# maxvonbuelow/harry

Measured on AMD Instinct MI355X. Metric: Mtriangles/s encode+decode, higher is better.
Workload: dtype u8/u16 residual bytes, u32 range-coder registers (compat profile: u64)

## Files before the change

### harry_amd/csrc/device/chunked.cpp

```cpp
#include <chrono>
#include <condition_variable>
#include <cstdio>
#include <cstdlib>
#include <cstring>
#include <deque>
#include <memory>
#include <mutex>
#include <thread>

#include "codec_math.hpp"
#include "context.hpp"
#include "kernels.hpp"

namespace hry {

using namespace dev;
static const char kMarkPrefix[] = "[hry enc]";

static constexpr int kDefaultChunk = 8192;
static constexpr uint32_t kMaxChunk = 1u << 20;


static uint32_t stream_words(uint32_t n, uint32_t t0)
{
// ... 596 lines not shown
	build_init_tables(m, kind_tabs);
	const uint32_t CHC = std::min(CH, std::max(CH / 8, 512u));
	dir.CH = CH; dir.CHC = CHC;
	const uint32_t npl = (uint32_t)planes.size();
	std::vector<HistSlice> slices;
	for (uint32_t pi = 0; pi < npl; ++pi)
		for (uint32_t f = 0; f < planes[pi].n; f += 16384) slices.push_back(HistSlice{ planes[pi].dptr + f, std::min(16384u, planes[pi].n - f), pi });
	cx.d_small.ensure(std::max<size_t>(slices.size() * sizeof(HistSlice) + (size_t)npl * 1024 + 64, 64));
	uint32_t *d_hist = cx.d_small.as<uint32_t>();
	HistSlice *d_slices = (HistSlice*)(cx.d_small.as<uint8_t>() + (size_t)npl * 1024);
	if (!slices.empty()) HIP_OK(hipMemcpyAsync(d_slices, slices.data(), slices.size() * sizeof(HistSlice), hipMemcpyHostToDevice, cx.stream));
	HIP_OK(hipMemsetAsync(d_hist, 0, (size_t)npl * 1024, cx.stream));
	HIP_OK(hipStreamSynchronize(cx.stream));
	cx.timing.h2d_ms = ms_since(t_h2d);
	HRY_MARK(t_all, "walk's outputs on the device");

	ConnView cv = cx.conn_view();
	HIP_OK(hipEventRecord(cx.ev[1], cx.stream));
	if (!m.general && !piped) {
		HIP_OK(hipMemsetAsync(cx.d_rank.p, 0xff, (size_t)dev_nv * 4, cx.stream));
		launch_rank(cx.stream, cx.d_order_v.as<uint32_t>(), vc, cv.org, cx.d_rank.as<uint32_t>());
		launch_predict_vtx(cx.stream, cv, cx.d_order_v.as<uint32_t>(), vc, cx.d_rank.as<uint32_t>(), cx.d_rec[1].as<uint8_t>(), ldv, cx.d_vplanes.as<uint8_t>());
		launch_face_planes(cx.stream, cv, cx.d_order_f.as<uint32_t>(), fc, cx.d_rec[0].as<uint8_t>(), ldf, cx.d_fplanes.as<uint8_t>());
	}
	split_conn_groups(cx, w, !nt_piped);
	{
		uint32_t base[8], o = 0;
		for (int k = 0; k < 8; ++k) { base[k] = o; o += (uint32_t)op_plane_n[k]; }
		cx.d_op.ensure(((nopb + kSplitUnit - 1) / kSplitUnit + 1) * 8 * 4 + 64);
		launch_split_classes(cx.stream, d_opraw, (uint32_t)nopb, base, cx.d_op.as<uint32_t>(), d_opplanes);
	}
	launch_plane_hist(cx.stream, d_slices, (uint32_t)slices.size(), d_hist);
	HIP_OK(hipEventRecord(cx.ev[2], cx.stream));
	std::vector<uint32_t> hist((size_t)npl * 256);
	if (npl) HIP_OK(hipMemcpyAsync(hist.data(), d_hist, hist.size() * 4, hipMemcpyDeviceToHost, cx.stream));
	HIP_OK(hipStreamSynchronize(cx.stream));
	HRY_MARK(t_all, "planes and their histograms");

	dir.tables.assign((size_t)npl * 256, 0);
	dir.has_prior.assign(npl, 0);
	dir.nsym.resize(npl);
	std::vector<uint32_t> totals(npl, 0);
	for (uint32_t pi = 0; pi < npl; ++pi) {
		uint32_t *tab = dir.tables.data() + (size_t)pi * 256;
		const bool use = plane_prior_from_hist(hist.data() + (size_t)pi * 256, planes[pi].n, tab);
		if (!use) memcpy(tab, kind_tabs.data() + (size_t)planes[pi].init * 256, 1024);
		for (int i = 0; i < 256; ++i) totals[pi] += tab[i];
		dir.has_prior[pi] = use ? 1 : 0;
		dir.nsym[pi] = planes[pi].n;
	}
	std::vector<StreamJob> jobs;
	uint64_t words = 0;
	uint64_t nsym_total = 0;
	uint32_t max_t0 = 256;
	for (uint32_t pi = 0; pi < npl; ++pi) {
		const PlaneRef &pl = planes[pi];
		nsym_total += pl.n;
		max_t0 = std::max(max_t0, totals[pi]);
		for_plane_streams(pi, pl.n, CH, CHC, [&](uint64_t f, uint32_t n) {
			if (words >= (1ull << 32) - (1u << 24)) throw Error(HRY_E_UNSUPPORTED, "chunked stream accumulator exceeds 2^32 words");
			jobs.push_back(StreamJob{ pl.dptr + f, n, pi, totals[pi], (uint32_t)words });
			words += stream_words(n, totals[pi]);
		});
	}
	const uint32_t ns = (uint32_t)jobs.size();
	const uint32_t nw = (uint32_t)words + 2;
	HRY_MARK(t_all, "  priors and stream jobs (host)");
	cx.d_init.ensure(std::max<size_t>(dir.tables.size() * 4, 16));
	if (!dir.tables.empty()) HIP_OK(hipMemcpyAsync(cx.d_init.p, dir.tables.data(), dir.tables.size() * 4, hipMemcpyHostToDevice, cx.stream));
	cx.d_cjobs.ensure(std::max<size_t>((size_t)ns * sizeof(StreamJob), 16));
	if (ns) HIP_OK(hipMemcpyAsync(cx.d_cjobs.p, jobs.data(), (size_t)ns * sizeof(StreamJob), hipMemcpyHostToDevice, cx.stream));
	cx.ensure_magic(max_t0 + CH + 16);
	cx.d_acc.ensure((size_t)nw * 8);
	cx.d_summary.ensure(((size_t)nw / 1024 + 8) * 4);
	cx.d_bytes.ensure((size_t)nw * 4);
	cx.d_csizes.ensure(std::max<size_t>((size_t)ns * 8, 16));
	cx.d_coffs.ensure(((size_t)ns + 1) * 8);
	HIP_OK(hipMemsetAsync(cx.d_acc.p, 0, (size_t)nw * 8, cx.stream));
	uint32_t *d_bits = cx.d_csizes.as<uint32_t>(), *d_nbytes = d_bits + ns;
	bool split_kernels;
	{
		uint32_t longest = 0;
		for (uint32_t i = 0; i < ns; ++i) longest = std::max(longest, jobs[i].n);
		const double one = std::max(longest * 0.09e-3, (double)nsym_total * 0.04e-6), two = longest * 0.207e-3 + (double)nsym_total * 0.0057e-6;
		const uint64_t min_streams = env_uint("HRY_ENCODE_SPLIT_MIN_STREAMS", ~0ull);
		split_kernels = min_streams != ~0ull ? min_streams != 0 && ns >= min_streams : ns >= 64 && two < 0.9 * one;
	}
	for (uint32_t i = 0; i < ns && split_kernels; ++i) split_kernels = (uint64_t)jobs[i].t0 + jobs[i].n <= 65535u;
	std::vector<uint64_t> tab;
	if (split_kernels) {
		tab.resize((size_t)ns + ((size_t)ns + 1) / 2);
		uint32_t *order = (uint32_t*)(tab.data() + ns);
		uint64_t off = 0;
		for (uint32_t i = 0; i < ns; ++i) { tab[i] = off; off += jobs[i].n; order[i] = i; }
		std::stable_sort(order, order + ns, [&](uint32_t a, uint32_t b) { return jobs[a].n > jobs[b].n; });
		cx.d_rec_sym.ensure(std::max<size_t>((size_t)off * 8, 16));
		cx.d_split.ensure(tab.size() * 8);
		HIP_OK(hipMemcpyAsync(cx.d_split.p, tab.data(), tab.size() * 8, hipMemcpyHostToDevice, cx.stream));
		HIP_OK(hipEventRecord(cx.ev[3], cx.stream));
		launch_chunk_encode_split(cx.stream, cx.d_cjobs.as<StreamJob>(), ns, cx.d_init.as<uint32_t>(), cx.d_magic.as<MagicEnt>(), cx.d_acc.as<uint64_t>(), d_bits,
		                          cx.d_split.as<uint64_t>(), cx.d_rec_sym.p, (const uint32_t*)(cx.d_split.as<uint64_t>() + ns));
		HIP_OK(hipEventRecord(cx.ev[4], cx.stream));
	} else {
	HIP_OK(hipEventRecord(cx.ev[3], cx.stream));
	launch_chunk_encode(cx.stream, cx.d_cjobs.as<StreamJob>(), ns, cx.d_init.as<uint32_t>(), cx.d_magic.as<MagicEnt>(), cx.d_acc.as<uint64_t>(), d_bits);
	HIP_OK(hipEventRecord(cx.ev[4], cx.stream));
	}
	launch_carry(cx.stream, cx.d_acc.as<uint64_t>(), nw, cx.d_v.as<uint64_t>(), cx.d_summary.as<uint32_t>(), cx.d_bytes.as<uint8_t>(), cx.d_cjobs.as<StreamJob>(), d_bits, ns);
	launch_stream_pack(cx.stream, cx.d_cjobs.as<StreamJob>(), ns, d_bits, nullptr, d_nbytes, cx.d_coffs.as<uint64_t>(), nullptr, false);
	cx.h_small.ensure(64);
	volatile uint64_t *total_bytes_p = cx.h_small.as<uint64_t>();
	*total_bytes_p = 0;
	HIP_OK(hipMemcpyAsync((void*)total_bytes_p, cx.d_coffs.as<uint64_t>() + ns, 8, hipMemcpyDeviceToHost, cx.stream));
	HRY_MARK(t_all, "  stream kernels launched");
	if (dir_beside) dir_helper.rethrow(); else select_restarts();
	HRY_MARK(t_all, "  restart points selected");
	HIP_OK(hipStreamSynchronize(cx.stream));
	const uint64_t total_bytes = *total_bytes_p;
	HRY_MARK(t_all, "streams coded");
	cx.d_cout.ensure(std::max<size_t>(total_bytes, 16));
	launch_stream_pack(cx.stream, cx.d_cjobs.as<StreamJob>(), ns, d_bits, cx.d_bytes.as<uint8_t>(), d_nbytes, cx.d_coffs.as<uint64_t>(), cx.d_cout.as<uint8_t>(), true);
	HIP_OK(hipEventRecord(cx.ev[5], cx.stream));

	write_container(cx, dir, restart_sec, ns, d_nbytes, total_bytes, out);
	HRY_MARK(t_all, "container on the host");
	if (sharded) { const uint64_t seg_len = out.size() - seg_begin; memcpy(out.data() + seg_len_at, &seg_len, 8); }
	if (cx.want_order) {
		if (sharded || in_place) throw Error(HRY_E_UNSUPPORTED, "HRY_FLAG_ORDER on a shard");
		order_build(cx, m, w, !piped ? cx.d_order_v.as<uint32_t>() : nullptr, !piped && (ldf.nplanes || m.general) ? cx.d_order_f.as<uint32_t>() : nullptr);
	}

	if (cx.keep_stages) {
		cx.stage_put_host("order_v", w.order_v.data(), (size_t)vc * 4);
		cx.stage_put_host("order_f", w.order_f.data(), (size_t)fc * 4);
		cx.stage_put("vplanes", cx.d_vplanes.p, (size_t)vc * ldv.nplanes);
		cx.stage_put("fplanes", cx.d_fplanes.p, (size_t)fc * ldf.nplanes);
		cx.stage_put("d_twin", cx.d_twin.p, (size_t)(in_place ? in_place->whole->ne() : m.ne()) * 4);
		uint64_t top = 0;
		for (uint32_t i = 0; i < ns; ++i) top = std::max(top, (uint64_t)jobs[i].t0 + jobs[i].n);
		const uint32_t plan[3] = { ns, split_kernels ? 1u : 0u, (uint32_t)top };
		cx.stage_put_host("enc_plan", plan, sizeof plan);
	}
	cx.timing.k_predict_ms = cx.elapsed(1, 2);
	cx.timing.k_entropy_ms = cx.elapsed(3, 4);
	cx.timing.device_ms = cx.elapsed(1, 5);
	cx.timing.n_symbols = nsym_total;
	cx.timing.payload_bytes = total_bytes;
	cx.timing.total_ms = ms_since(t_all);
}

Mesh *decode_chunked(Context &cx, const uint8_t *p, size_t n, size_t hdr, std::unique_ptr<Mesh> m);
Mesh *decode_compat(Context &cx, const uint8_t *p, size_t n, size_t hdr, std::unique_ptr<Mesh> m);

Mesh *decode_any(Context &cx, const uint8_t *p, size_t n, int shard_index, int shard_count, bool allow_partial)
{
	HIP_OK(hipSetDevice(cx.device));
	std::unique_ptr<Mesh> m(new Mesh());
	int minor = 0;
	const bool sharded = n >= 6 && p[4] == 0 && p[5] == 3;
	size_t hdr = read_hry_header(p, n, *m, minor, !sharded);
	if (minor == 3) { Context *one = &cx; return decode_sharded(&one, 1, p, n, hdr, std::move(m), shard_index, shard_count, allow_partial || shard_count > 1, nullptr); }
	if (shard_count > 1) throw Error(HRY_E_ARG, "only a sharded container (.hry v0.3) decodes segment by segment");
	if (minor == 2) return decode_chunked(cx, p, n, hdr, std::move(m));
	if (m->general) return decode_general(cx, p, n, hdr, std::move(m));
	return decode_compat(cx, p, n, hdr, std::move(m));
}

// ... 2 lines not shown
```

### harry_amd/csrc/device/chunked.hip

```cpp
#include <hip/hip_runtime.h>

#include <mutex>
#include <stdexcept>
#include <type_traits>

#include "codec_math.hpp"
#include "dev_types.hpp"
#include "kernels.hpp"
#include "wave.hpp"

namespace hry {
namespace dev {

constexpr int kWin = 72;

__global__ __launch_bounds__(64) void k_chunk_encode(const StreamJob *jobs, const uint32_t *inits, const MagicEnt *magic,
                                                     unsigned long long *acc, uint32_t *stream_bits)
{
	const StreamJob jb = jobs[blockIdx.x];
	const int lane = threadIdx.x;
	__shared__ uint32_t cnt[257], cum[257], bh[256];
	__shared__ unsigned long long win[kWin];
	{
		const uint32_t *st = inits + (size_t)jb.init * 256 + 4 * lane;
		uint32_t a = st[0], b = st[1], c = st[2], d = st[3], tot;
		uint32_t ex = wave_excl_scan(a + b + c + d, tot);
		cnt[4 * lane] = a; cnt[4 * lane + 1] = b; cnt[4 * lane + 2] = c; cnt[4 * lane + 3] = d;
		cum[4 * lane] = ex; cum[4 * lane + 1] = ex + a; cum[4 * lane + 2] = ex + a + b; cum[4 * lane + 3] = ex + a + b + c;
		if (lane == 0) { cnt[256] = 0; cum[256] = 0; }
	}
	__syncthreads();
	uint32_t R = 1u << 31;
	uint32_t S = 0;
	const uint64_t earlier = lane == 0 ? 0ull : (~0ull >> (64 - lane));
	for (uint32_t base = 0; base < jb.n; base += 64) {
		const uint32_t j = base + lane;
		const bool valid = j < jb.n;
		const uint32_t nb = min(64u, jb.n - base);
		const uint32_t s = valid ? jb.sym[j] : 0x100u;
		uint64_t eq = ~0ull, lt = 0;
#pragma unroll
		for (int b = 8; b >= 0; --b) {
			const bool mine = (s >> b) & 1u;
			const uint64_t m = __ballot(mine);
			lt |= mine ? (eq & ~m) : 0ull;
			eq &= mine ? m : ~m;
		}
		const uint32_t l = cum[s] + (uint32_t)__popcll(lt & earlier), c = cnt[s] + (uint32_t)__popcll(eq & earlier);
		const uint32_t t = jb.t0 + j;
		const bool sub = l + c == t;
		MagicEnt me = valid ? magic[t] : MagicEnt{ 0, 0, 0 };
		const uint32_t mx = valid ? (sub ? l : c) : 0u;
		const uint32_t mm = ((me.shift >> kMagicSh32Shift) & 31u) | (sub || !valid ? 0x80u : 0u);
		uint32_t my_r = 0, my_s = 0;
		const uint32_t s_first = S;
		auto step = [&](uint32_t i) {
			const uint32_t M = (uint32_t)__builtin_amdgcn_readlane((int)me.m32, (int)i);
			const uint32_t x = (uint32_t)__builtin_amdgcn_readlane((int)mx, (int)i);
			const uint32_t meta = (uint32_t)__builtin_amdgcn_readlane((int)mm, (int)i);
			const uint32_t r = __umulhi(R, M) >> (meta & 31u);
			const uint32_t prod = r * x;
			const uint32_t Rn = (meta & 0x80u) ? R - prod : prod;
			const uint32_t y = Rn - 1u;
			const uint32_t sh = y ? (uint32_t)__builtin_clz(y) - 1u : 31u;
			my_r = lane == (int)i ? r : my_r;
			my_s = lane == (int)i ? S : my_s;
			R = Rn << sh;
			S += sh;
		};
		uint32_t i = 0;
		for (; i + 4 <= nb; i += 4) { step(i); step(i + 1); step(i + 2); step(i + 3); }
		for (; i < nb; ++i) step(i);
		const uint32_t w0 = s_first >> 5, span = ((S + 63) >> 5) - w0 + 1;
		const uint32_t a = (valid && l) ? my_r * l : 0u;
		const uint32_t w = my_s >> 5, shb = my_s & 31;
		const uint32_t hi = a >> shb, lo = shb ? a << (32 - shb) : 0u;
		unsigned long long *dst = acc + jb.word_base;
		for (uint32_t k = lane; k < span; k += 64) win[k] = 0;
		bh[4 * lane] = 0; bh[4 * lane + 1] = 0; bh[4 * lane + 2] = 0; bh[4 * lane + 3] = 0;
		__syncthreads();
		if (hi) atomicAdd(&win[w - w0], (unsigned long long)hi);
		if (lo) atomicAdd(&win[w - w0 + 1], (unsigned long long)lo);
		if (valid) atomicAdd(&bh[s], 1u);
		__syncthreads();
		for (uint32_t k = lane; k < span; k += 64) {
			unsigned long long v = win[k];
			if (v) atomicAdd(&dst[w0 + k], v);
		}
		uint32_t a0 = bh[4 * lane], a1 = bh[4 * lane + 1], a2 = bh[4 * lane + 2], a3 = bh[4 * lane + 3], tot;
		uint32_t ex = wave_excl_scan(a0 + a1 + a2 + a3, tot);
		cnt[4 * lane] += a0; cnt[4 * lane + 1] += a1; cnt[4 * lane + 2] += a2; cnt[4 * lane + 3] += a3;
		cum[4 * lane] += ex; cum[4 * lane + 1] += ex + a0; cum[4 * lane + 2] += ex + a0 + a1; cum[4 * lane + 3] += ex + a0 + a1 + a2;
		__syncthreads();
	}
	if (lane == 0) stream_bits[blockIdx.x] = S + 32;
}

__global__ __launch_bounds__(64) void k_chunk_model(const StreamJob *jobs, const uint32_t *inits, const MagicEnt *magic, const unsigned long long *rec_off, uint2 *rec)
{
	const StreamJob jb = jobs[blockIdx.x];
	const int lane = threadIdx.x;
	__shared__ uint32_t cnt[257], cum[257], bh[256];
	{
		const uint32_t *st = inits + (size_t)jb.init * 256 + 4 * lane;
		uint32_t a = st[0], b = st[1], c = st[2], d = st[3], tot;
		uint32_t ex = wave_excl_scan(a + b + c + d, tot);
		cnt[4 * lane] = a; cnt[4 * lane + 1] = b; cnt[4 * lane + 2] = c; cnt[4 * lane + 3] = d;
		cum[4 * lane] = ex; cum[4 * lane + 1] = ex + a; cum[4 * lane + 2] = ex + a + b; cum[4 * lane + 3] = ex + a + b + c;
		if (lane == 0) { cnt[256] = 0; cum[256] = 0; }
	}
	__syncthreads();
	uint2 *out = rec + rec_off[blockIdx.x];
	const uint64_t earlier = lane == 0 ? 0ull : (~0ull >> (64 - lane));
	for (uint32_t base = 0; base < jb.n; base += 64) {
		const uint32_t j = base + lane;
		const bool valid = j < jb.n;
		const uint32_t s = valid ? jb.sym[j] : 0x100u;
		uint64_t eq = ~0ull, lt = 0;
#pragma unroll
		for (int b = 8; b >= 0; --b) {
			const bool mine = (s >> b) & 1u;
			const uint64_t m = __ballot(mine);
			lt |= mine ? (eq & ~m) : 0ull;
			eq &= mine ? m : ~m;
		}
		const uint32_t l = cum[s] + (uint32_t)__popcll(lt & earlier), c = cnt[s] + (uint32_t)__popcll(eq & earlier);
		if (valid) {
			const MagicEnt me = magic[jb.t0 + j];
			const uint32_t msh = (me.shift >> kMagicSh32Shift) & 31u;
			const uint32_t q = me.m32 == 0x80000000u ? me.m32 >> msh : (me.m32 - 1u) >> msh;
			out[j] = make_uint2(l | (c << 16), q);
		}
		bh[4 * lane] = 0; bh[4 * lane + 1] = 0; bh[4 * lane + 2] = 0; bh[4 * lane + 3] = 0;
		__syncthreads();
		if (valid) atomicAdd(&bh[s], 1u);
		__syncthreads();
		uint32_t a0 = bh[4 * lane], a1 = bh[4 * lane + 1], a2 = bh[4 * lane + 2], a3 = bh[4 * lane + 3], tot;
		uint32_t ex = wave_excl_scan(a0 + a1 + a2 + a3, tot);
		cnt[4 * lane] += a0; cnt[4 * lane + 1] += a1; cnt[4 * lane + 2] += a2; cnt[4 * lane + 3] += a3;
		cum[4 * lane] += ex; cum[4 * lane + 1] += ex + a0; cum[4 * lane + 2] += ex + a0 + a1; cum[4 * lane + 3] += ex + a0 + a1 + a2;
		__syncthreads();
	}
}

__global__ __launch_bounds__(64) void k_chunk_ranges(const StreamJob *jobs, uint32_t njobs, const uint32_t *order, const unsigned long long *rec_off,
                                                     const uint2 *rec, unsigned long long *acc, uint32_t *stream_bits)
{
	__shared__ uint32_t tile_lc[64 * 65], tile_q[64 * 65];
	const uint32_t lane = threadIdx.x;
	const uint32_t slot = blockIdx.x * 64 + lane;
	const bool have = slot < njobs;
	const uint32_t job = have ? order[slot] : 0u;
	StreamJob jb{ nullptr, 0, 0, 256, 0 };
	if (have) jb = jobs[job];
	const uint32_t n = have ? jb.n : 0u;
	const uint2 *in = rec + (have ? rec_off[job] : 0ull);
	unsigned long long *dst = acc + jb.word_base;
	const uint32_t nmax = (uint32_t)__builtin_amdgcn_readfirstlane((int)wave_max(n));
	const uint32_t in_lo = (uint32_t)(uintptr_t)in, in_hi = (uint32_t)((uintptr_t)in >> 32);
	uint2 nxt[64];
	auto fetch = [&](uint32_t step0) {
#pragma unroll
		for (int s = 0; s < 64; ++s) {
			const uint32_t ns = (uint32_t)__builtin_amdgcn_readlane((int)n, s);
			const uint2 *ps = (const uint2*)(((uintptr_t)(uint32_t)__builtin_amdgcn_readlane((int)in_hi, s) << 32) | (uint32_t)__builtin_amdgcn_readlane((int)in_lo, s));
			const uint32_t j = step0 + lane;
			nxt[s] = j < ns ? ps[j] : make_uint2(0u, 0u);
		}
	};
	auto stash = [&]() {
#pragma unroll
		for (int s = 0; s < 64; ++s) { tile_lc[s * 65 + lane] = nxt[s].x; tile_q[s * 65 + lane] = nxt[s].y; }
	};
	uint32_t R = 1u << 31, S = 0, t = jb.t0;
	uint32_t cur_w = 0;
	unsigned long long a0 = 0, a1 = 0;
	fetch(0);
	stash();
	for (uint32_t step0 = 0; step0 < nmax; step0 += 64) {
		const bool more = step0 + 64 < nmax;
		if (more) fetch(step0 + 64);
		const uint32_t *row_lc = tile_lc + lane * 65, *row_q = tile_q + lane * 65;
		const uint32_t left = nmax - step0 < 64u ? nmax - step0 : 64u;
		for (uint32_t k = 0; k < left; ++k) {
			const uint32_t lc = row_lc[k], q = row_q[k];
			const bool live = step0 + k < n;
			const uint32_t l = lc & 0xffffu, c = lc >> 16;
			uint32_t r = __umulhi(R, q);
			r += R - r * t >= t ? 1u : 0u;
			uint32_t rl, rc;
			asm("v_mul_lo_u32 %0, %1, %2" : "=v"(rl) : "v"(r), "v"(l));
			asm("v_mul_lo_u32 %0, %1, %2" : "=v"(rc) : "v"(r), "v"(c));
			const uint32_t Rn = l + c == t ? R - rl : rc;
			const uint32_t w = S >> 5;
			const unsigned long long two = ((unsigned long long)(live ? rl : 0u) << 32) >> (S & 31u);
			if (w != cur_w) { dst[cur_w] = a0; a0 = a1; a1 = 0; cur_w = w; }
			a0 += two >> 32;
			a1 += two & 0xffffffffull;
			const uint32_t y = Rn - 1u;
			const uint32_t sh = y ? (uint32_t)__builtin_clz(y) - 1u : 31u;
			R = live ? Rn << sh : R;
			S += live ? sh : 0u;
			t += live ? 1u : 0u;
		}
		if (more) stash();
	}
	if (have) {
		dst[cur_w] = a0;
		dst[cur_w + 1u] = a1;
		stream_bits[job] = S + 32u;
	}
}

__global__ __launch_bounds__(1024) void k_stream_offsets(const uint32_t *stream_bits, uint32_t n, uint32_t *nbytes, unsigned long long *offsets)
{
	__shared__ unsigned long long s_wave[17];
	unsigned long long carry = 0;
	for (uint32_t base = 0; base < n; base += 1024) {
		const uint32_t i = base + threadIdx.x;
		const uint32_t nb = i < n ? (stream_bits[i] + 7) >> 3 : 0;
		unsigned long long total;
		const unsigned long long ex = block_excl_scan<unsigned long long>(nb, s_wave, total);
		if (i < n) { nbytes[i] = nb; offsets[i] = carry + ex; }
		carry += total;
		__syncthreads();
	}
	if (threadIdx.x == 0) offsets[n] = carry;
}

__global__ __launch_bounds__(256) void k_pack_streams(const StreamJob *jobs, const uint8_t *bytes, const uint32_t *nbytes, const unsigned long long *offsets, uint8_t *out)
{
	const StreamJob jb = jobs[blockIdx.x];
	const uint8_t *src = bytes + (size_t)jb.word_base * 4;
	uint8_t *dst = out + offsets[blockIdx.x];
	for (uint32_t i = threadIdx.x; i < nbytes[blockIdx.x]; i += 256) dst[i] = src[i];
}

__global__ __launch_bounds__(256) void k_scatter_u8(const uint8_t *src, const uint32_t *dst_index, uint32_t n, uint8_t *dst)
{
	uint32_t i = blockIdx.x * blockDim.x + threadIdx.x;
	if (i < n) dst[dst_index[i]] = src[i];
}

__global__ __launch_bounds__(64) void k_chunk_decode(const StreamJob *jobs, const uint32_t *inits, const MagicEnt *magic,
                                                     const uint8_t *payload, const unsigned long long *offsets, const uint32_t *nbytes, uint8_t *sym_out_base)
{
	const StreamJob jb = jobs[blockIdx.x];
	const int lane = threadIdx.x;
	uint8_t *out = const_cast<uint8_t*>(jb.sym);
	(void)sym_out_base;
	uint32_t i0, i1, i2, i3, sym_last;
	{
		const uint32_t *st = inits + (size_t)jb.init * 256 + 4 * lane;
		const uint32_t c0 = st[0], c1 = st[1], c2 = st[2], c3 = st[3];
		uint32_t tot, ex = wave_excl_scan(c0 + c1 + c2 + c3, tot);
		i0 = ex + c0; i1 = i0 + c1; i2 = i1 + c2; i3 = i2 + c3;
		const uint32_t top = c3 ? 4 * lane + 3 : c2 ? 4 * lane + 2 : c1 ? 4 * lane + 1 : c0 ? 4 * lane : 0u;
		sym_last = (uint32_t)__builtin_amdgcn_readfirstlane((int)wave_max(top));
	}
	const uint8_t *src = payload + offsets[blockIdx.x];
	const uint32_t nby = nbytes[blockIdx.x];
	auto byte_at = [&](uint32_t k) -> uint32_t { return k < nby ? src[k] : 0xffu; };
	uint32_t D = (byte_at(0) << 24) | (byte_at(1) << 16) | (byte_at(2) << 8) | byte_at(3);
	D = (uint32_t)__builtin_amdgcn_readfirstlane((int)D);
	uint32_t pos = 32;
	uint32_t R = 1u << 31;
	for (uint32_t base = 0; base < jb.n; base += 64) {
		const uint32_t nb = min(64u, jb.n - base);
		const MagicEnt me = base + lane < jb.n ? magic[jb.t0 + base + lane] : MagicEnt{ 0, 0, 0 };
		const uint32_t msh = (me.shift >> kMagicSh32Shift) & 31u;
		const uint32_t wbyte = pos >> 3;
		const uint32_t kb = wbyte + 4 * lane;
		uint32_t wword;
		if (kb + 4 <= nby) { uint32_t raw; __builtin_memcpy(&raw, src + kb, 4); wword = __builtin_bswap32(raw); }
		else wword = (byte_at(kb) << 24) | (byte_at(kb + 1) << 16) | (byte_at(kb + 2) << 8) | byte_at(kb + 3);
		uint32_t wo = pos & 7u;
		uint32_t mysym = 0;
		auto run = [&](auto use24) {
			for (uint32_t i = 0; i < nb; ++i) {
				const uint32_t t = jb.t0 + base + i;
				const uint32_t M = (uint32_t)__builtin_amdgcn_readlane((int)me.m32, (int)i);
				const uint32_t shf = (uint32_t)__builtin_amdgcn_readlane((int)msh, (int)i);
				const uint32_t r = __umulhi(R, M) >> shf;
				uint32_t p0, p1, p2, p3;
				if constexpr (decltype(use24)::value) { p0 = __umul24(i0, r); p1 = __umul24(i1, r); p2 = __umul24(i2, r); p3 = __umul24(i3, r); }
				else { p0 = i0 * r; p1 = i1 * r; p2 = i2 * r; p3 = i3 * r; }
				const uint64_t b0 = __ballot(p0 <= D), b1 = __ballot(p1 <= D), b2 = __ballot(p2 <= D), b3 = __ballot(p3 <= D);
				const uint32_t below = (uint32_t)(__popcll(b0) + __popcll(b1) + __popcll(b2) + __popcll(b3));
				const uint32_t s = min(below, sym_last);
				const uint32_t ls = s >> 2, k = s & 3u;
				const uint32_t e0 = (uint32_t)__builtin_amdgcn_readlane((int)p0, (int)ls), e1 = (uint32_t)__builtin_amdgcn_readlane((int)p1, (int)ls);
				const uint32_t e2 = (uint32_t)__builtin_amdgcn_readlane((int)p2, (int)ls), e3 = (uint32_t)__builtin_amdgcn_readlane((int)p3, (int)ls);
				const uint32_t pv = (uint32_t)__builtin_amdgcn_readlane((int)p3, (int)(ls ? ls - 1 : 0));
				const uint32_t rh = k == 0 ? e0 : k == 1 ? e1 : k == 2 ? e2 : e3;
				const uint32_t rl = k == 0 ? (ls ? pv : 0u) : k == 1 ? e0 : k == 2 ? e1 : e2;
				const uint32_t Rn = s < sym_last ? rh - rl : R - rl;
				const uint32_t y = Rn - 1u;
				const uint32_t sh = y ? (uint32_t)__builtin_clz(y) - 1u : 31u;
				R = Rn << sh;
				const uint32_t wk = wo >> 5, wb = wo & 31u;
				const uint64_t two = ((uint64_t)(uint32_t)__builtin_amdgcn_readlane((int)wword, (int)wk) << 32) |
				                     (uint64_t)(uint32_t)__builtin_amdgcn_readlane((int)wword, (int)min(wk + 1u, 63u));
				const uint32_t bits = (uint32_t)(((two << wb) >> 1) >> (63u - sh));
				D = ((D - rl) << sh) | bits;
				wo += sh;
				const uint32_t e = 4 * lane;
				i0 += (e >= s); i1 += (e + 1 >= s); i2 += (e + 2 >= s); i3 += (e + 3 >= s);
				mysym = lane == (int)i ? s : mysym;
				(void)t;
			}
		};
		if (jb.t0 + base > 128u) run(std::true_type()); else run(std::false_type());
		pos = 8 * wbyte + wo;
		if (base + lane < jb.n) out[base + lane] = (uint8_t)mysym;
	}
}

template <typename CT>
__global__ __launch_bounds__(64) void k_chunk_decode_lanes(const StreamJob *jobs, uint32_t njobs, const uint32_t *inits, const MagicEnt *magic,
                                                           const uint8_t *payload, const unsigned long long *offsets, const uint32_t *nbytes)
{
	extern __shared__ uint32_t lds_tab[];
	CT *const cnt = (CT*)lds_tab;
	const uint32_t lane = threadIdx.x;
	const uint32_t j = blockIdx.x * 64 + lane;
	const bool have = j < njobs;
	StreamJob jb{ nullptr, 0, 0, 256, 0 };
	if (have) jb = jobs[j];
	uint32_t C[16];
	{
		const uint32_t *st = inits + (size_t)jb.init * 256;
		uint32_t sum = 0;
#pragma unroll
		for (int b = 0; b < 16; ++b) {
#pragma unroll
			for (int k = 0; k < 16; ++k) {
				const uint32_t c = have ? st[b * 16 + k] : 0u;
				cnt[(b * 16 + k) * 64 + lane] = (CT)c;
				sum += c;
			}
			C[b] = sum;
		}
	}
	const uint8_t *src = payload + (have ? offsets[j] : 0ull);
	const uint32_t nby = have ? nbytes[j] : 0u;
	auto byte_at = [&](uint32_t k) -> uint32_t { return k < nby ? src[k] : 0xffu; };
	auto word_at = [&](uint32_t k) -> uint32_t {
		if (k + 4 <= nby) { uint32_t raw; __builtin_memcpy(&raw, src + k, 4); return __builtin_bswap32(raw); }
		return (byte_at(k) << 24) | (byte_at(k + 1) << 16) | (byte_at(k + 2) << 8) | byte_at(k + 3);
	};
	uint32_t D = word_at(0);
	uint32_t p = 8;
	uint32_t ahead = word_at(4);
	uint64_t buf = 0;
	uint32_t avail = 0;
	uint32_t R = 1u << 31, t = jb.t0;
	typedef __attribute__((address_space(1))) uint8_t gbyte;
	gbyte *out = (gbyte*)const_cast<uint8_t*>(jb.sym);
	const uint32_t nmax = (uint32_t)__builtin_amdgcn_readfirstlane((int)wave_max(jb.n));
	MagicEnt me = magic[t];
	uint32_t o0 = 0, o1 = 0, o2 = 0, o3 = 0;
	for (uint32_t i = 0; i < nmax; ++i) {
		if ((i & 15u) == 0u && i) {
			if (i < jb.n) {
				typedef uint32_t u32x4 __attribute__((ext_vector_type(4)));
				typedef __attribute__((address_space(1))) u32x4 __attribute__((aligned(1))) gvec;
				*(gvec*)(out + i - 16) = u32x4{ o0, o1, o2, o3 };
			}
		}
		if (i >= jb.n) continue;
		const uint32_t r = __umulhi(R, me.m32) >> ((me.shift >> kMagicSh32Shift) & 31u);
		me = magic[t + 1u];
		uint32_t q = (uint32_t)((float)D * __builtin_amdgcn_rcpf((float)r));
		int32_t rem = (int32_t)(D - __umul24(q, r));
		if (rem < 0) { --q; rem += (int32_t)r; }
		if (rem < 0) { --q; rem += (int32_t)r; }
		if (rem >= (int32_t)r) { ++q; rem -= (int32_t)r; }
		if (rem >= (int32_t)r) { ++q; rem -= (int32_t)r; }
		const uint32_t target = min(t - 1u, q);
		uint32_t b = 0, lo = 0;
#pragma unroll
		for (int k = 0; k < 16; ++k) {
			const bool le = C[k] <= target;
			b += le ? 1u : 0u;
			lo = le ? C[k] : lo;
		}
		const CT *cb = cnt + (size_t)(b * 16u) * 64 + lane;
		uint32_t sin = 0, run = lo, hi = 0xffffffffu;
#pragma unroll
		for (int k = 0; k < 16; ++k) {
			run += (uint32_t)cb[k * 64];
			const bool le = run <= target;
			sin += le ? 1u : 0u;
			lo = le ? run : lo;
			hi = min(hi, le ? 0xffffffffu : run);
		}
// ... 30 lines not shown
}

__global__ __launch_bounds__(256) void k_plane_hist(const HistSlice *slices, uint32_t *hist)
{
	const HistSlice sl = slices[blockIdx.x];
	__shared__ uint32_t bins[256];
	bins[threadIdx.x] = 0;
	__syncthreads();
	for (uint32_t i = threadIdx.x; i < sl.n; i += 256) atomicAdd(&bins[sl.sym[i]], 1u);
	__syncthreads();
	if (bins[threadIdx.x]) atomicAdd(&hist[(size_t)sl.plane * 256 + threadIdx.x], bins[threadIdx.x]);
}

__global__ __launch_bounds__(64) void k_split_count(const uint8_t *ops, uint32_t n, uint32_t *cnt)
{
	const uint32_t u = blockIdx.x, lane = threadIdx.x;
	uint32_t c[8] = { 0, 0, 0, 0, 0, 0, 0, 0 };
	for (uint32_t i = u * kSplitUnit + lane; i < min(n, (u + 1) * kSplitUnit); i += 64) {
		const uint32_t k = ops[i] >> 3;
#pragma unroll
		for (int j = 0; j < 8; ++j) c[j] += k == (uint32_t)j;
	}
#pragma unroll
	for (int j = 0; j < 8; ++j) {
		const uint32_t v = wave_sum(c[j]);
		if (lane == 0) cnt[u * 8 + j] = v;
	}
}
__global__ __launch_bounds__(64) void k_split_scan(uint32_t *cnt, uint32_t nunits, SplitBase base)
{
	const uint32_t j = blockIdx.x, lane = threadIdx.x;
	uint32_t run = base.b[j];
	for (uint32_t u0 = 0; u0 < nunits; u0 += 64) {
		const uint32_t u = u0 + lane;
		const uint32_t c = u < nunits ? cnt[u * 8 + j] : 0u;
		uint32_t tot;
		const uint32_t ex = wave_excl_scan(c, tot);
		if (u < nunits) cnt[u * 8 + j] = run + ex;
		run += tot;
	}
}
__global__ __launch_bounds__(64) void k_split_place(const uint8_t *ops, uint32_t n, const uint32_t *cnt, uint8_t *planes)
{
	const uint32_t u = blockIdx.x, lane = threadIdx.x;
	uint32_t at[8];
#pragma unroll
	for (int j = 0; j < 8; ++j) at[j] = cnt[u * 8 + j];
	const uint32_t end = min(n, (u + 1) * kSplitUnit);
	for (uint32_t i0 = u * kSplitUnit; i0 < end; i0 += 64) {
		const uint32_t i = i0 + lane;
		const bool live = i < end;
		const uint32_t b = live ? ops[i] : 0xffu, k = b >> 3;
		uint32_t dst = 0;
#pragma unroll
		for (int j = 0; j < 8; ++j) {
			const uint64_t mk = __ballot(live && k == (uint32_t)j);
			if (live && k == (uint32_t)j) dst = at[j] + (uint32_t)__popcll(mk & ((1ull << lane) - 1ull));
			at[j] += (uint32_t)__popcll(mk);
		}
		if (live) planes[dst] = (uint8_t)(b & 7u);
	}
}
void launch_split_classes(hipStream_t st, const uint8_t *ops, uint32_t n, const uint32_t base[8], uint32_t *scratch, uint8_t *planes)
{
	if (!n) return;
	const uint32_t nunits = (n + kSplitUnit - 1) / kSplitUnit;
	SplitBase sb;
	for (int j = 0; j < 8; ++j) sb.b[j] = base[j];
	hipLaunchKernelGGL(k_split_count, dim3(nunits), dim3(64), 0, st, ops, n, scratch);
	hipLaunchKernelGGL(k_split_scan, dim3(8), dim3(64), 0, st, scratch, nunits, sb);
	hipLaunchKernelGGL(k_split_place, dim3(nunits), dim3(64), 0, st, ops, n, scratch, planes);
}

void launch_plane_hist(hipStream_t st, const HistSlice *slices, uint32_t nslices, uint32_t *hist)
{
	if (nslices) hipLaunchKernelGGL(k_plane_hist, dim3(nslices), dim3(256), 0, st, slices, hist);
}
void launch_scatter_u32(hipStream_t st, const uint32_t *pairs, uint32_t n, uint32_t *dst)
{
	if (n) hipLaunchKernelGGL(k_scatter_u32, dim3((n + 255) / 256), dim3(256), 0, st, pairs, n, dst);
}
void launch_chunk_encode(hipStream_t st, const StreamJob *jobs, uint32_t nstreams, const uint32_t *inits, const MagicEnt *magic, uint64_t *acc, uint32_t *stream_bits)
{
	if (nstreams) hipLaunchKernelGGL(k_chunk_encode, dim3(nstreams), dim3(64), 0, st, jobs, inits, magic, (unsigned long long*)acc, stream_bits);
}
void launch_chunk_encode_split(hipStream_t st, const StreamJob *jobs, uint32_t nstreams, const uint32_t *inits, const MagicEnt *magic, uint64_t *acc, uint32_t *stream_bits,
                               const uint64_t *rec_off, void *rec, const uint32_t *order)
{
	if (!nstreams) return;
	hipLaunchKernelGGL(k_chunk_model, dim3(nstreams), dim3(64), 0, st, jobs, inits, magic, (const unsigned long long*)rec_off, (uint2*)rec);
	hipLaunchKernelGGL(k_chunk_ranges, dim3((nstreams + 63) / 64), dim3(64), 0, st, jobs, nstreams, order, (const unsigned long long*)rec_off, (const uint2*)rec,
	                   (unsigned long long*)acc, stream_bits);
}
void launch_stream_pack(hipStream_t st, const StreamJob *jobs, uint32_t nstreams, const uint32_t *stream_bits, const uint8_t *bytes,
                        uint32_t *nbytes, uint64_t *offsets, uint8_t *out, bool pack)
{
	if (!pack) hipLaunchKernelGGL(k_stream_offsets, dim3(1), dim3(1024), 0, st, stream_bits, nstreams, nbytes, (unsigned long long*)offsets);
	else if (nstreams) hipLaunchKernelGGL(k_pack_streams, dim3(nstreams), dim3(256), 0, st, jobs, bytes, nbytes, (const unsigned long long*)offsets, out);
}
void launch_scatter_u8(hipStream_t st, const uint8_t *src, const uint32_t *dst_index, uint32_t n, uint8_t *dst)
{
	if (n) hipLaunchKernelGGL(k_scatter_u8, dim3((n + 255) / 256), dim3(256), 0, st, src, dst_index, n, dst);
}
void launch_chunk_decode(hipStream_t st, const StreamJob *jobs, uint32_t nstreams, const uint32_t *inits, const MagicEnt *magic,
                         const uint8_t *payload, const uint64_t *offsets, const uint32_t *nbytes)
{
	if (nstreams) hipLaunchKernelGGL(k_chunk_decode, dim3(nstreams), dim3(64), 0, st, jobs, inits, magic, payload, (const unsigned long long*)offsets, nbytes, (uint8_t*)nullptr);
}
template <typename CT>
static void launch_chunk_decode_lanes_as(hipStream_t st, const StreamJob *jobs, uint32_t nstreams, const uint32_t *inits, const MagicEnt *magic,
                                         const uint8_t *payload, const uint64_t *offsets, const uint32_t *nbytes)
{
	constexpr uint32_t kLds = 256 * 64 * sizeof(CT);
	static std::mutex mu;
	static bool raised[64] = {};
	int dev = 0;
	if (hipGetDevice(&dev) != hipSuccess || dev < 0 || dev >= 64) dev = 0;
	{
		std::lock_guard<std::mutex> g(mu);
		if (!raised[dev]) {
			if (hipFuncSetAttribute((const void*)k_chunk_decode_lanes<CT>, hipFuncAttributeMaxDynamicSharedMemorySize, (int)kLds) != hipSuccess) {
				(void)hipGetLastError();
				throw std::runtime_error("k_chunk_decode_lanes: the device refuses its dynamic LDS");
			}
			raised[dev] = true;
		}
	}
	hipLaunchKernelGGL(k_chunk_decode_lanes<CT>, dim3((nstreams + 63) / 64), dim3(64), kLds, st, jobs, nstreams, inits, magic, payload, (const unsigned long long*)offsets, nbytes);
	if (hipGetLastError() != hipSuccess) throw std::runtime_error("k_chunk_decode_lanes: launch failed");
}
void launch_chunk_decode_lanes(hipStream_t st, const StreamJob *jobs, uint32_t nstreams, const uint32_t *inits, const MagicEnt *magic,
                               const uint8_t *payload, const uint64_t *offsets, const uint32_t *nbytes, bool counts16)
{
	if (!nstreams) return;
	if (counts16) launch_chunk_decode_lanes_as<uint16_t>(st, jobs, nstreams, inits, magic, payload, offsets, nbytes);
	else launch_chunk_decode_lanes_as<uint32_t>(st, jobs, nstreams, inits, magic, payload, offsets, nbytes);
}

}
}
```

Before: 62.21.

## Pipeline chunk encode across modeller/coder waves and streamline decode symbol search

The chunk encoder now runs two waves per block. One wave builds the adaptive model for batch k and writes packed operands to double-buffered LDS, while the other runs the serial range-coding steps for batch k-1, so the modelling work overlaps the serial chain. The decoder replaces its popcount-and-readlane symbol search with a single owner lookup via ctz and DPP, keeps a 64-bit bit buffer instead of re-reading two words each step, and updates counts with carry-add inline asm. The split-kernel heuristic constants are also retuned. The risks are a mix of wave-scope fences with block barriers, the packed x field limited to 21 bits, and inline-asm correctness.

```diff
diff --git a/harry_amd/csrc/device/chunked.cpp b/harry_amd/csrc/device/chunked.cpp
--- a/harry_amd/csrc/device/chunked.cpp
+++ b/harry_amd/csrc/device/chunked.cpp
@@ -702,7 +702,7 @@
 	{
 		uint32_t longest = 0;
 		for (uint32_t i = 0; i < ns; ++i) longest = std::max(longest, jobs[i].n);
-		const double one = std::max(longest * 0.09e-3, (double)nsym_total * 0.04e-6), two = longest * 0.207e-3 + (double)nsym_total * 0.0057e-6;
+		const double one = std::max(longest * 0.073e-3, (double)nsym_total * 0.049e-6), two = longest * 0.207e-3 + (double)nsym_total * 0.0057e-6;
 		const uint64_t min_streams = env_uint("HRY_ENCODE_SPLIT_MIN_STREAMS", ~0ull);
 		split_kernels = min_streams != ~0ull ? min_streams != 0 && ns >= min_streams : ns >= 64 && two < 0.9 * one;
 	}
diff --git a/harry_amd/csrc/device/chunked.hip b/harry_amd/csrc/device/chunked.hip
--- a/harry_amd/csrc/device/chunked.hip
+++ b/harry_amd/csrc/device/chunked.hip
@@ -14,87 +14,108 @@
 
 constexpr int kWin = 72;
 
-__global__ __launch_bounds__(64) void k_chunk_encode(const StreamJob *jobs, const uint32_t *inits, const MagicEnt *magic,
-                                                     unsigned long long *acc, uint32_t *stream_bits)
+#define HRY_WAVE_LDS_ORDER() do { __builtin_amdgcn_fence(__ATOMIC_SEQ_CST, "wavefront"); __builtin_amdgcn_wave_barrier(); } while (0)
+__global__ __launch_bounds__(128) void k_chunk_encode(const StreamJob *jobs, const uint32_t *inits, const MagicEnt *magic,
+                                                      unsigned long long *acc, uint32_t *stream_bits)
 {
 	const StreamJob jb = jobs[blockIdx.x];
-	const int lane = threadIdx.x;
+	const int lane = threadIdx.x & 63;
+	const bool modeller = __builtin_amdgcn_readfirstlane((int)(threadIdx.x >> 6)) != 0;
 	__shared__ uint32_t cnt[257], cum[257], bh[256];
 	__shared__ unsigned long long win[kWin];
-	{
+	__shared__ uint32_t op_m[2][64], op_x[2][64], op_l[2][64];
+	const uint32_t nbatch = (jb.n + 63) >> 6;
+	const uint64_t earlier = lane == 0 ? 0ull : (~0ull >> (64 - lane));
+	uint32_t s_next = 0x100u;
+	MagicEnt me_next{ 0, 0, 0 };
+	if (modeller) {
 		const uint32_t *st = inits + (size_t)jb.init * 256 + 4 * lane;
 		uint32_t a = st[0], b = st[1], c = st[2], d = st[3], tot;
 		uint32_t ex = wave_excl_scan(a + b + c + d, tot);
 		cnt[4 * lane] = a; cnt[4 * lane + 1] = b; cnt[4 * lane + 2] = c; cnt[4 * lane + 3] = d;
 		cum[4 * lane] = ex; cum[4 * lane + 1] = ex + a; cum[4 * lane + 2] = ex + a + b; cum[4 * lane + 3] = ex + a + b + c;
 		if (lane == 0) { cnt[256] = 0; cum[256] = 0; }
-	}
-	__syncthreads();
+		if ((uint32_t)lane < jb.n) { s_next = jb.sym[lane]; me_next = magic[jb.t0 + lane]; }
+		HRY_WAVE_LDS_ORDER();
+	}
 	uint32_t R = 1u << 31;
 	uint32_t S = 0;
-	const uint64_t earlier = lane == 0 ? 0ull : (~0ull >> (64 - lane));
-	for (uint32_t base = 0; base < jb.n; base += 64) {
-		const uint32_t j = base + lane;
-		const bool valid = j < jb.n;
-		const uint32_t nb = min(64u, jb.n - base);
-		const uint32_t s = valid ? jb.sym[j] : 0x100u;
-		uint64_t eq = ~0ull, lt = 0;
-#pragma unroll
-		for (int b = 8; b >= 0; --b) {
-			const bool mine = (s >> b) & 1u;
-			const uint64_t m = __ballot(mine);
-			lt |= mine ? (eq & ~m) : 0ull;
-			eq &= mine ? m : ~m;
-		}
-		const uint32_t l = cum[s] + (uint32_t)__popcll(lt & earlier), c = cnt[s] + (uint32_t)__popcll(eq & earlier);
-		const uint32_t t = jb.t0 + j;
-		const bool sub = l + c == t;
-		MagicEnt me = valid ? magic[t] : MagicEnt{ 0, 0, 0 };
-		const uint32_t mx = valid ? (sub ? l : c) : 0u;
-		const uint32_t mm = ((me.shift >> kMagicSh32Shift) & 31u) | (sub || !valid ? 0x80u : 0u);
-		uint32_t my_r = 0, my_s = 0;
-		const uint32_t s_first = S;
-		auto step = [&](uint32_t i) {
-			const uint32_t M = (uint32_t)__builtin_amdgcn_readlane((int)me.m32, (int)i);
-			const uint32_t x = (uint32_t)__builtin_amdgcn_readlane((int)mx, (int)i);
-			const uint32_t meta = (uint32_t)__builtin_amdgcn_readlane((int)mm, (int)i);
-			const uint32_t r = __umulhi(R, M) >> (meta & 31u);
-			const uint32_t prod = r * x;
-			const uint32_t Rn = (meta & 0x80u) ? R - prod : prod;
-			const uint32_t y = Rn - 1u;
-			const uint32_t sh = y ? (uint32_t)__builtin_clz(y) - 1u : 31u;
-			my_r = lane == (int)i ? r : my_r;
-			my_s = lane == (int)i ? S : my_s;
-			R = Rn << sh;
-			S += sh;
-		};
-		uint32_t i = 0;
-		for (; i + 4 <= nb; i += 4) { step(i); step(i + 1); step(i + 2); step(i + 3); }
-		for (; i < nb; ++i) step(i);
-		const uint32_t w0 = s_first >> 5, span = ((S + 63) >> 5) - w0 + 1;
-		const uint32_t a = (valid && l) ? my_r * l : 0u;
-		const uint32_t w = my_s >> 5, shb = my_s & 31;
-		const uint32_t hi = a >> shb, lo = shb ? a << (32 - shb) : 0u;
-		unsigned long long *dst = acc + jb.word_base;
-		for (uint32_t k = lane; k < span; k += 64) win[k] = 0;
-		bh[4 * lane] = 0; bh[4 * lane + 1] = 0; bh[4 * lane + 2] = 0; bh[4 * lane + 3] = 0;
+	for (uint32_t k = 0; k <= nbatch; ++k) {
+		if (modeller) {
+			if (k < nbatch) {
+				const uint32_t j = k * 64 + lane;
+				const bool valid = j < jb.n;
+				const uint32_t s = valid ? s_next : 0x100u;
+				const MagicEnt me = me_next;
+				if (j + 64 < jb.n) { s_next = jb.sym[j + 64]; me_next = magic[jb.t0 + j + 64]; }
+				uint64_t eq = ~0ull, lt = 0;
+#pragma unroll
+				for (int b = 8; b >= 0; --b) {
+					const bool mine = (s >> b) & 1u;
+					const uint64_t m = __ballot(mine);
+					lt |= mine ? (eq & ~m) : 0ull;
+					eq &= mine ? m : ~m;
+				}
+				const uint32_t l = cum[s] + (uint32_t)__popcll(lt & earlier), c = cnt[s] + (uint32_t)__popcll(eq & earlier);
+				const uint32_t t = jb.t0 + j;
+				const bool sub = l + c == t;
+				const uint32_t mx = valid ? (sub ? l : c) : 0u;
+				op_m[k & 1][lane] = me.m32;
+				op_x[k & 1][lane] = ((me.shift >> kMagicSh32Shift) & 31u) | (mx << 5) | (sub || !valid ? 0x80000000u : 0u);
+				op_l[k & 1][lane] = valid ? l : 0u;
+				bh[4 * lane] = 0; bh[4 * lane + 1] = 0; bh[4 * lane + 2] = 0; bh[4 * lane + 3] = 0;
+				HRY_WAVE_LDS_ORDER();
+				if (valid) atomicAdd(&bh[s], 1u);
+				HRY_WAVE_LDS_ORDER();
+				uint32_t a0 = bh[4 * lane], a1 = bh[4 * lane + 1], a2 = bh[4 * lane + 2], a3 = bh[4 * lane + 3], tot;
+				uint32_t ex = wave_excl_scan(a0 + a1 + a2 + a3, tot);
+				cnt[4 * lane] += a0; cnt[4 * lane + 1] += a1; cnt[4 * lane + 2] += a2; cnt[4 * lane + 3] += a3;
+				cum[4 * lane] += ex; cum[4 * lane + 1] += ex + a0; cum[4 * lane + 2] += ex + a0 + a1; cum[4 * lane + 3] += ex + a0 + a1 + a2;
+				HRY_WAVE_LDS_ORDER();
+			}
+		} else if (k > 0) {
+			const uint32_t base = (k - 1) * 64;
+			const uint32_t nb = min(64u, jb.n - base);
+			const uint32_t m32 = op_m[(k - 1) & 1][lane], xm = op_x[(k - 1) & 1][lane], l = op_l[(k - 1) & 1][lane];
+			uint32_t my_r = 0, my_s = 0;
+			const uint32_t s_first = S;
+			auto step = [&](uint32_t i) {
+				const uint32_t M = (uint32_t)__builtin_amdgcn_readlane((int)m32, (int)i);
+				const uint32_t meta = (uint32_t)__builtin_amdgcn_readlane((int)xm, (int)i);
+				const uint32_t r = __umulhi(R, M) >> (meta & 31u);
+				const uint32_t prod = r * ((meta >> 5) & 0x1fffffu);
+				const uint32_t Rn = (int32_t)meta < 0 ? R - prod : prod;
+				const uint32_t y = Rn - 1u;
+				const uint32_t sh = y ? (uint32_t)__builtin_clz(y) - 1u : 31u;
+				my_r = lane == (int)i ? r : my_r;
+				my_s = lane == (int)i ? S : my_s;
+				R = Rn << sh;
+				S += sh;
+			};
+			uint32_t i = 0;
+			for (; i + 4 <= nb; i += 4) { step(i); step(i + 1); step(i + 2); step(i + 3); }
+			for (; i < nb; ++i) step(i);
+			const uint32_t w0 = s_first >> 5, span = ((S + 63) >> 5) - w0 + 1;
+			const uint32_t a = (uint32_t)lane < nb && l ? my_r * l : 0u;
+			const uint32_t w = my_s >> 5, shb = my_s & 31;
+			const uint32_t hi = a >> shb, lo = shb ? a << (32 - shb) : 0u;
+			unsigned long long *dst = acc + jb.word_base;
+			for (uint32_t q = lane; q < span; q += 64) win[q] = 0;
+			HRY_WAVE_LDS_ORDER();
+			if (hi) atomicAdd(&win[w - w0], (unsigned long long)hi);
+			if (lo) atomicAdd(&win[w - w0 + 1], (unsigned long long)lo);
+			HRY_WAVE_LDS_ORDER();
+			for (uint32_t q = lane; q < span; q += 64) {
+				unsigned long long v = win[q];
+				if (v) atomicAdd(&dst[w0 + q], v);
+			}
+			HRY_WAVE_LDS_ORDER();
+		}
 		__syncthreads();
-		if (hi) atomicAdd(&win[w - w0], (unsigned long long)hi);
-		if (lo) atomicAdd(&win[w - w0 + 1], (unsigned long long)lo);
-		if (valid) atomicAdd(&bh[s], 1u);
-		__syncthreads();
-		for (uint32_t k = lane; k < span; k += 64) {
-			unsigned long long v = win[k];
-			if (v) atomicAdd(&dst[w0 + k], v);
-		}
-		uint32_t a0 = bh[4 * lane], a1 = bh[4 * lane + 1], a2 = bh[4 * lane + 2], a3 = bh[4 * lane + 3], tot;
-		uint32_t ex = wave_excl_scan(a0 + a1 + a2 + a3, tot);
-		cnt[4 * lane] += a0; cnt[4 * lane + 1] += a1; cnt[4 * lane + 2] += a2; cnt[4 * lane + 3] += a3;
-		cum[4 * lane] += ex; cum[4 * lane + 1] += ex + a0; cum[4 * lane + 2] += ex + a0 + a1; cum[4 * lane + 3] += ex + a0 + a1 + a2;
-		__syncthreads();
-	}
-	if (lane == 0) stream_bits[blockIdx.x] = S + 32;
-}
+	}
+	if (threadIdx.x == 0) stream_bits[blockIdx.x] = S + 32;
+}
+#undef HRY_WAVE_LDS_ORDER
 
 __global__ __launch_bounds__(64) void k_chunk_model(const StreamJob *jobs, const uint32_t *inits, const MagicEnt *magic, const unsigned long long *rec_off, uint2 *rec)
 {
@@ -242,6 +263,13 @@
 	if (i < n) dst[dst_index[i]] = src[i];
 }
 
+__device__ __forceinline__ void add_bits(uint32_t &a, uint64_t ma, uint32_t &b, uint64_t mb, uint32_t &c, uint64_t mc, uint32_t &d, uint64_t md)
+{
+	uint64_t carry_out;
+	asm("v_addc_co_u32 %0, %4, 0, %0, %5\n\tv_addc_co_u32 %1, %4, 0, %1, %6\n\tv_addc_co_u32 %2, %4, 0, %2, %7\n\tv_addc_co_u32 %3, %4, 0, %3, %8"
+	    : "+v"(a), "+v"(b), "+v"(c), "+v"(d), "=&s"(carry_out) : "s"(ma), "s"(mb), "s"(mc), "s"(md));
+}
+
 __global__ __launch_bounds__(64) void k_chunk_decode(const StreamJob *jobs, const uint32_t *inits, const MagicEnt *magic,
                                                      const uint8_t *payload, const unsigned long long *offsets, const uint32_t *nbytes, uint8_t *sym_out_base)
 {
@@ -258,6 +286,9 @@
 		const uint32_t top = c3 ? 4 * lane + 3 : c2 ? 4 * lane + 2 : c1 ? 4 * lane + 1 : c0 ? 4 * lane : 0u;
 		sym_last = (uint32_t)__builtin_amdgcn_readfirstlane((int)wave_max(top));
 	}
+	const uint32_t e = 4 * lane;
+	const uint32_t k0 = e < sym_last ? 0u : 0x7fffffffu, k1 = e + 1 < sym_last ? 0u : 0x7fffffffu;
+	const uint32_t k2 = e + 2 < sym_last ? 0u : 0x7fffffffu, k3 = e + 3 < sym_last ? 0u : 0x7fffffffu;
 	const uint8_t *src = payload + offsets[blockIdx.x];
 	const uint32_t nby = nbytes[blockIdx.x];
 	auto byte_at = [&](uint32_t k) -> uint32_t { return k < nby ? src[k] : 0xffu; };
@@ -274,44 +305,46 @@
 		uint32_t wword;
 		if (kb + 4 <= nby) { uint32_t raw; __builtin_memcpy(&raw, src + kb, 4); wword = __builtin_bswap32(raw); }
 		else wword = (byte_at(kb) << 24) | (byte_at(kb + 1) << 16) | (byte_at(kb + 2) << 8) | byte_at(kb + 3);
-		uint32_t wo = pos & 7u;
+		const uint32_t wo = pos & 7u;
+		uint64_t buf = (((uint64_t)(uint32_t)__builtin_amdgcn_readlane((int)wword, 0) << 32) | (uint32_t)__builtin_amdgcn_readlane((int)wword, 1)) << wo;
+		uint32_t avail = 64u - wo, nextw = 2;
 		uint32_t mysym = 0;
 		auto run = [&](auto use24) {
 			for (uint32_t i = 0; i < nb; ++i) {
-				const uint32_t t = jb.t0 + base + i;
 				const uint32_t M = (uint32_t)__builtin_amdgcn_readlane((int)me.m32, (int)i);
 				const uint32_t shf = (uint32_t)__builtin_amdgcn_readlane((int)msh, (int)i);
 				const uint32_t r = __umulhi(R, M) >> shf;
 				uint32_t p0, p1, p2, p3;
-				if constexpr (decltype(use24)::value) { p0 = __umul24(i0, r); p1 = __umul24(i1, r); p2 = __umul24(i2, r); p3 = __umul24(i3, r); }
-				else { p0 = i0 * r; p1 = i1 * r; p2 = i2 * r; p3 = i3 * r; }
-				const uint64_t b0 = __ballot(p0 <= D), b1 = __ballot(p1 <= D), b2 = __ballot(p2 <= D), b3 = __ballot(p3 <= D);
-				const uint32_t below = (uint32_t)(__popcll(b0) + __popcll(b1) + __popcll(b2) + __popcll(b3));
-				const uint32_t s = min(below, sym_last);
-				const uint32_t ls = s >> 2, k = s & 3u;
-				const uint32_t e0 = (uint32_t)__builtin_amdgcn_readlane((int)p0, (int)ls), e1 = (uint32_t)__builtin_amdgcn_readlane((int)p1, (int)ls);
-				const uint32_t e2 = (uint32_t)__builtin_amdgcn_readlane((int)p2, (int)ls), e3 = (uint32_t)__builtin_amdgcn_readlane((int)p3, (int)ls);
-				const uint32_t pv = (uint32_t)__builtin_amdgcn_readlane((int)p3, (int)(ls ? ls - 1 : 0));
-				const uint32_t rh = k == 0 ? e0 : k == 1 ? e1 : k == 2 ? e2 : e3;
-				const uint32_t rl = k == 0 ? (ls ? pv : 0u) : k == 1 ? e0 : k == 2 ? e1 : e2;
+				if constexpr (decltype(use24)::value) { p0 = __umul24(i0, r) + k0; p1 = __umul24(i1, r) + k1; p2 = __umul24(i2, r) + k2; p3 = __umul24(i3, r) + k3; }
+				else { p0 = i0 * r + k0; p1 = i1 * r + k1; p2 = i2 * r + k2; p3 = i3 * r + k3; }
+				const bool g0 = p0 > D, g1 = p1 > D, g2 = p2 > D, g3 = p3 > D;
+				const uint64_t m0 = __ballot(g0), m1 = __ballot(g1), m2 = __ballot(g2), m3 = __ballot(g3);
+				const uint32_t owner = (uint32_t)__builtin_ctzll(m3);
+				const uint32_t left = (uint32_t)__builtin_amdgcn_update_dpp(0, (int)p3, 0x138 , 0xf, 0xf, true);
+				const uint32_t my_h = g0 ? p0 : g1 ? p1 : g2 ? p2 : p3;
+				const uint32_t my_l = g0 ? left : g1 ? p0 : g2 ? p1 : p2;
+				const uint32_t my_c = g0 ? 0u : g1 ? 1u : g2 ? 2u : 3u;
+				const uint32_t s = 4u * owner + (uint32_t)__builtin_amdgcn_readlane((int)my_c, (int)owner);
+				const uint32_t rl = (uint32_t)__builtin_amdgcn_readlane((int)my_l, (int)owner);
+				const uint32_t rh = (uint32_t)__builtin_amdgcn_readlane((int)my_h, (int)owner);
 				const uint32_t Rn = s < sym_last ? rh - rl : R - rl;
 				const uint32_t y = Rn - 1u;
 				const uint32_t sh = y ? (uint32_t)__builtin_clz(y) - 1u : 31u;
 				R = Rn << sh;
-				const uint32_t wk = wo >> 5, wb = wo & 31u;
-				const uint64_t two = ((uint64_t)(uint32_t)__builtin_amdgcn_readlane((int)wword, (int)wk) << 32) |
-				                     (uint64_t)(uint32_t)__builtin_amdgcn_readlane((int)wword, (int)min(wk + 1u, 63u));
-				const uint32_t bits = (uint32_t)(((two << wb) >> 1) >> (63u - sh));
-				D = ((D - rl) << sh) | bits;
-				wo += sh;
-				const uint32_t e = 4 * lane;
-				i0 += (e >= s); i1 += (e + 1 >= s); i2 += (e + 2 >= s); i3 += (e + 3 >= s);
+				D = (uint32_t)(((((uint64_t)(D - rl)) << 32 | (uint32_t)(buf >> 32)) << sh) >> 32);
+				buf <<= sh;
+				avail -= sh;
+				if (avail < 32u) {
+					buf |= (uint64_t)(uint32_t)__builtin_amdgcn_readlane((int)wword, (int)(nextw & 63u)) << (32u - avail);
+					avail += 32u;
+					++nextw;
+				}
+				add_bits(i0, m0, i1, m1, i2, m2, i3, m3);
 				mysym = lane == (int)i ? s : mysym;
-				(void)t;
 			}
 		};
 		if (jb.t0 + base > 128u) run(std::true_type()); else run(std::false_type());
-		pos = 8 * wbyte + wo;
+		pos = 8 * wbyte + 32u * nextw - avail;
 		if (base + lane < jb.n) out[base + lane] = (uint8_t)mysym;
 	}
 }
@@ -508,7 +541,7 @@
 }
 void launch_chunk_encode(hipStream_t st, const StreamJob *jobs, uint32_t nstreams, const uint32_t *inits, const MagicEnt *magic, uint64_t *acc, uint32_t *stream_bits)
 {
-	if (nstreams) hipLaunchKernelGGL(k_chunk_encode, dim3(nstreams), dim3(64), 0, st, jobs, inits, magic, (unsigned long long*)acc, stream_bits);
+	if (nstreams) hipLaunchKernelGGL(k_chunk_encode, dim3(nstreams), dim3(128), 0, st, jobs, inits, magic, (unsigned long long*)acc, stream_bits);
 }
 void launch_chunk_encode_split(hipStream_t st, const StreamJob *jobs, uint32_t nstreams, const uint32_t *inits, const MagicEnt *magic, uint64_t *acc, uint32_t *stream_bits,
                                const uint64_t *rec_off, void *rec, const uint32_t *order)
```

Result: faster. 63.24, median of 6 (+1.7%).
